# shuoshuof/Humanoid-Real-Time-Retarget

Measured on AMD Instinct MI355X. Metric: retargeted frames/sec + max joint-angle err vs ref, Hu humanoid @1/2/4/8 GPU, higher is better.
Workload: dtype f32; 1 GPU; VtrdynFullBodyPosRetargeter batched solve, Hu v5 target (BASELINE config 3); global_batch=262144, parallelism=dp1, input_layout=soa, input_ring_sets=3, precise_gripper=True, launch=K plain launches, step i on stream i % 2

## Files before the change

humanoid-real-time-retarget_amd/csrc/rtg_knobs.h:

```cpp
#pragma once

#ifndef RTG_SIDES_TILES
#define RTG_SIDES_TILES 2
#endif
#ifndef RTG_SIDES_EARLY_WORDS
#define RTG_SIDES_EARLY_WORDS 1
#endif
#ifndef RTG_AOS_PRELOAD_TIPS
#define RTG_AOS_PRELOAD_TIPS 1
#endif
#ifndef RTG_SIDES_SOA_WAVES
#define RTG_SIDES_SOA_WAVES 5
#endif
#ifndef RTG_SIDES_UNIFORM_WAVE
#define RTG_SIDES_UNIFORM_WAVE 3
#endif
#ifndef RTG_QUAD8_MAX_B
#define RTG_QUAD8_MAX_B 2048
#endif
#ifndef RTG_QUAD_MAX_B
#define RTG_QUAD_MAX_B 4096
#endif
#ifndef RTG_LATENCY_MAX_B
#define RTG_LATENCY_MAX_B 49152
#endif
#ifndef RTG_EXP_HOT_INPUTS
#define RTG_EXP_HOT_INPUTS 0
#endif
#ifndef RTG_EXP_TIMESTAMPS
#define RTG_EXP_TIMESTAMPS 0
#endif
#ifndef RTG_EXP_SKIP_SIGNAL
#define RTG_EXP_SKIP_SIGNAL 0
#endif
#ifndef RTG_VEL_SEG
#define RTG_VEL_SEG 10
#endif
#ifndef RTG_VEL_LDS_MIN
#define RTG_VEL_LDS_MIN 0
#endif
#ifndef RTG_FK_NT_OUT
#define RTG_FK_NT_OUT 1
#endif
#ifndef RTG_FK_F16_MAXJ
#define RTG_FK_F16_MAXJ 36
#endif
#ifndef RTG_EXP_MULR_NOBRANCH
#define RTG_EXP_MULR_NOBRANCH 0
#endif
#ifndef RTG_EXP_NO_TABLE
#define RTG_EXP_NO_TABLE 0
#endif
#ifndef RTG_TORSO_X0
#define RTG_TORSO_X0 1
#endif
#ifndef RTG_FIT_FAST_DIV
#define RTG_FIT_FAST_DIV 1
#endif
#ifndef RTG_FIT_FAST_DIV_TU
#define RTG_FIT_FAST_DIV_TU RTG_FIT_FAST_DIV
#endif
#ifndef RTG_FDIV_CORRECTIONS
#define RTG_FDIV_CORRECTIONS 1
#endif
#if RTG_FDIV_CORRECTIONS != 1 && RTG_FDIV_CORRECTIONS != 2
#error "RTG_FDIV_CORRECTIONS: 1 or 2 (fewer gives wrong quotients)"
#endif
#ifndef RTG_DOF_NT_STORE
#define RTG_DOF_NT_STORE 1
#endif
#ifndef RTG_VEL_W
#define RTG_VEL_W 8
#endif
#ifndef RTG_DOF_NWAY
#define RTG_DOF_NWAY 4
#endif
#ifndef RTG_UNIT_TAB_K
#define RTG_UNIT_TAB_K 16
#endif
#ifndef RTG_SIDES_SHARED_FIT
#define RTG_SIDES_SHARED_FIT 1
#endif
#ifndef RTG_EULER_LIBM
#define RTG_EULER_LIBM 1
#endif
#ifndef RTG_UPPER_UNIT_TAB
#define RTG_UPPER_UNIT_TAB 1
#endif
#ifndef RTG_ROT_UNIT_TAB
#define RTG_ROT_UNIT_TAB 1
#endif
#ifndef RTG_SIDES_UNIT_TAB
#define RTG_SIDES_UNIT_TAB 7
#endif
#ifndef RTG_SIDES_UNIT_TAB_AOS
#define RTG_SIDES_UNIT_TAB_AOS 1
#endif
#ifndef RTG_FRAME1_UNIT_TAB
#define RTG_FRAME1_UNIT_TAB 6
#endif
#ifndef RTG_FK_UNIT_TAB
#define RTG_FK_UNIT_TAB 1
#endif
#ifndef RTG_DOF_UNIT_TAB
#define RTG_DOF_UNIT_TAB 1
#endif
#ifndef RTG_VEL_UNIT_TAB
#define RTG_VEL_UNIT_TAB 1
#endif
#ifndef RTG_VEL_ANG_NB
#define RTG_VEL_ANG_NB 2
#endif
#ifndef RTG_ROT_INGEST_TILE_AOS
#define RTG_ROT_INGEST_TILE_AOS 16
#endif
#ifndef RTG_ROT_INGEST_TILE_SOA
#define RTG_ROT_INGEST_TILE_SOA 16
#endif
#ifndef RTG_EXP_NO_RARE
#define RTG_EXP_NO_RARE 0
#endif
#ifndef RTG_EXP_STUB_SVD
#define RTG_EXP_STUB_SVD 0
#endif
```

humanoid-real-time-retarget_amd/csrc/rtg_ops.hip:

```cpp
#include "rtg_device.cuh"

namespace rtg {

struct Dir3 {
    float x, y, z;
    int32_t on;
};

__global__ __launch_bounds__(256) void k_rescale_motion(TopoView T, const float *__restrict__ motion, int64_t B,
                                                        Dir3 dir, float *__restrict__ out)
{
    const int64_t f = (int64_t)blockIdx.x * blockDim.x + threadIdx.x;
    if (f >= B) return;
    const int J = T.J;
    const float *m = motion + f * J * 3;
    float *o = out + f * J * 3;
    auto mp = [&](int j) {
        const V v = ld3(m + 3 * j);
        return dir.on ? V{v.x * dir.x, v.y * dir.y, v.z * dir.z} : v;
    };
    for (int j = 0; j < J; ++j) {
        const int p = ld_const(T.parents + j);
        const V mj = mp(j);
        if (p < 0) {
// ... 760 lines not shown
    for (int i = 0; i < 20; ++i) {
#pragma unroll
        for (int c = 0; c < 3; ++c) {
            lh[lay_idx(soa, f, i, c, 20, 3, B)] = jit(14 + i, c);
            rh[lay_idx(soa, f, i, c, 20, 3, B)] = jit(39 + i, c);
        }
    }
}

hipError_t launch_rescale_motion(const TopoView &T, const float *motion, int64_t B, const float *dir, float *out,
                                 hipStream_t s)
{
    const Dir3 d = dir ? Dir3{dir[0], dir[1], dir[2], 1} : Dir3{1.0f, 1.0f, 1.0f, 0};
    hipLaunchKernelGGL(k_rescale_motion, dim3(grid_for(B, 256)), dim3(256), 0, s, T, motion, B, d, out);
    return hipGetLastError();
}

hipError_t launch_quat_between(const float *v1, const float *v2, int64_t n, float *out, float *ws, hipStream_t s)
{
    hipError_t e = hipMemsetAsync(ws, 0, 2 * sizeof(float), s);
    if (e != hipSuccess) return e;
    hipLaunchKernelGGL(k_qbtv_norm_max, dim3(grid_for(n, 256)), dim3(256), 0, s, v1, v2, n, ws);
    hipLaunchKernelGGL(k_quat_between, dim3(grid_for(n, 256)), dim3(256), 0, s, v1, v2, n, ws, out);
    return hipGetLastError();
}

hipError_t launch_rebuild_vtrdyn(const TopoView &T, const float *motion, int64_t B, float *g_rot, float *root_t,
                                 float *ws, hipStream_t s)
{
    hipError_t e = hipMemsetAsync(ws, 0, T.J * sizeof(float), s);
    if (e != hipSuccess) return e;
    hipLaunchKernelGGL(k_rebuild_norm_max, dim3(grid_for(B, 256)), dim3(256), 0, s, T, motion, B, ws);
    hipLaunchKernelGGL(k_rebuild_vtrdyn, dim3(grid_for(B, 256)), dim3(256), 0, s, T, motion, B, ws, g_rot, root_t);
    return hipGetLastError();
}

hipError_t launch_ingest_vtrdyn(const float *bp, const float *lhp, const float *rhp, int64_t B, int layout,
                                float *body, float *lh, float *rh, uint8_t *valid, hipStream_t s)
{
    if (layout == RTG_LAYOUT_SOA)
        hipLaunchKernelGGL(k_ingest_vtrdyn<kIngSoaTile>, dim3(grid_for(B, kIngSoaTile)), dim3(256), 0, s, bp,
                           lhp, rhp, B, body, lh, rh, valid, true);
    else
        hipLaunchKernelGGL(k_ingest_vtrdyn<kIngAosTile>, dim3(grid_for(B, kIngAosTile)), dim3(256), 0, s, bp,
                           lhp, rhp, B, body, lh, rh, valid, false);
    return hipGetLastError();
}

hipError_t launch_quat_op(int op, const float *a, const float *b, const float *c, int64_t n, float *out,
                          hipStream_t s)
{
    hipLaunchKernelGGL(k_quat_op, dim3(grid_for(n, 256)), dim3(256), 0, s, op, a, b, c, n, out);
    return hipGetLastError();
}

hipError_t launch_cal_joint_quat(const float *Z, const float *M, int npts, int64_t n, float *out, hipStream_t s)
{
    const dim3 g(grid_for(n, 256)), b(256);
    switch (npts) {
    case 1: hipLaunchKernelGGL(k_cal_joint_quat<1>, g, b, 0, s, Z, M, n, out); break;
    case 2: hipLaunchKernelGGL(k_cal_joint_quat<2>, g, b, 0, s, Z, M, n, out); break;
    case 3: hipLaunchKernelGGL(k_cal_joint_quat<3>, g, b, 0, s, Z, M, n, out); break;
    case 4: hipLaunchKernelGGL(k_cal_joint_quat<4>, g, b, 0, s, Z, M, n, out); break;
    case 5: hipLaunchKernelGGL(k_cal_joint_quat<5>, g, b, 0, s, Z, M, n, out); break;
    case 6: hipLaunchKernelGGL(k_cal_joint_quat<6>, g, b, 0, s, Z, M, n, out); break;
    case 7: hipLaunchKernelGGL(k_cal_joint_quat<7>, g, b, 0, s, Z, M, n, out); break;
    default: hipLaunchKernelGGL(k_cal_joint_quat<8>, g, b, 0, s, Z, M, n, out); break;
    }
    return hipGetLastError();
}

hipError_t launch_quat_as_euler(const float *q, int s0, int s1, int s2, int extrinsic, int degrees, int64_t n,
                               double *out, hipStream_t s)
{
    hipLaunchKernelGGL(k_quat_as_euler, dim3(grid_for(n, 256)), dim3(256), 0, s, q, s0, s1, s2, extrinsic, degrees, n,
                       out);
    return hipGetLastError();
}
hipError_t launch_quat_in_xyz_axis(const float *q, int s0, int s1, int s2, int extrinsic, int64_t n, float *out,
                                   hipStream_t s)
{
    hipLaunchKernelGGL(k_quat_in_xyz_axis, dim3(grid_for(n, 256)), dim3(256), 0, s, q, s0, s1, s2, extrinsic, n, out);
    return hipGetLastError();
}

hipError_t launch_synth_full_body(const TopoView &T, uint64_t seed, int64_t off, int64_t B, float *body, float *lh,
                                  float *rh, float *body_rot, int layout, hipStream_t s)
{
    hipLaunchKernelGGL(k_synth_full_body, dim3(grid_for(B, 64)), dim3(64), 0, s, T, seed, off, B, body, lh, rh,
                       body_rot,
                       layout == RTG_LAYOUT_SOA);
    return hipGetLastError();
}

constexpr int kProbeIters = 4096;
__global__ __launch_bounds__(256) void k_probe_valu(float seed, float *__restrict__ sink, uint64_t *__restrict__ clk)
{
    float a[8];
#pragma unroll
    for (int k = 0; k < 8; ++k) a[k] = seed + (float)(threadIdx.x + k);
    const bool rec = (blockIdx.x & 63) == 0 && threadIdx.x == 0;
    uint64_t c0 = 0, w0 = 0;
    if (rec) {
        c0 = clock64();
        w0 = wall_clock64();
    }
    for (int i = 0; i < kProbeIters; ++i) {
#pragma unroll
        for (int k = 0; k < 8; ++k) a[k] = __builtin_fmaf(a[k], 0.999999f, 1e-7f);
    }
    if (rec) {
        const uint64_t c1 = clock64(), w1 = wall_clock64();
        clk[2 * (blockIdx.x >> 6)] = c1 - c0;
        clk[2 * (blockIdx.x >> 6) + 1] = w1 - w0;
    }
    float s = 0.0f;
#pragma unroll
    for (int k = 0; k < 8; ++k) s += a[k];
    if (s == 12345.678f) sink[threadIdx.x] = s;
}
__global__ __launch_bounds__(256) void k_probe_copy(const float4 *__restrict__ src, float4 *__restrict__ dst,
                                                    int64_t n)
{
    for (int64_t i = (int64_t)blockIdx.x * 256 + threadIdx.x; i < n; i += (int64_t)gridDim.x * 256) dst[i] = src[i];
}

hipError_t launch_probe_valu(int nblocks, float *sink, uint64_t *clk, hipStream_t s)
{
    hipLaunchKernelGGL(k_probe_valu, dim3(nblocks), dim3(256), 0, s, 1.0f, sink, clk);
    return hipGetLastError();
}
hipError_t launch_probe_copy(const float *src, float *dst, int64_t nfloat4, hipStream_t s)
{
    hipLaunchKernelGGL(k_probe_copy, dim3(256 * 32), dim3(256), 0, s, reinterpret_cast<const float4 *>(src),
                       reinterpret_cast<float4 *>(dst), nfloat4);
    return hipGetLastError();
}
int probe_valu_iters() { return kProbeIters; }

}

#if RTG_EXP_STUB_SVD + RTG_EXP_NO_TABLE + RTG_EXP_HOT_INPUTS + RTG_EXP_MULR_NOBRANCH + RTG_EXP_NO_RARE + \
    RTG_EXP_TIMESTAMPS + RTG_EXP_SKIP_SIGNAL == 0
#define RTG_WRONG_ANSWER_KNOBS 0
#else
#define RTG_WRONG_ANSWER_KNOBS 1
#endif
#define RTG_STR2(x) #x
#define RTG_STR(x) RTG_STR2(x)
#define RTG_KNOB(k) "\"" #k "\":\"" RTG_STR(k) "\","
extern "C" const char *rtg_build_info(void)
{
    return "{\"abi\":" RTG_STR(RTG_ABI_VERSION) ",\"arch\":\"gfx950\",\"knobs\":{"
        RTG_KNOB(RTG_DOF_NWAY) RTG_KNOB(RTG_DOF_UNIT_TAB) RTG_KNOB(RTG_FK_UNIT_TAB) RTG_KNOB(RTG_UNIT_TAB_K) RTG_KNOB(RTG_SIDES_SHARED_FIT) RTG_KNOB(RTG_UPPER_UNIT_TAB) RTG_KNOB(RTG_ROT_UNIT_TAB) RTG_KNOB(RTG_EULER_LIBM) RTG_KNOB(RTG_SIDES_UNIT_TAB) RTG_KNOB(RTG_SIDES_UNIT_TAB_AOS) RTG_KNOB(RTG_FRAME1_UNIT_TAB) RTG_KNOB(RTG_VEL_UNIT_TAB) RTG_KNOB(RTG_SIDES_SOA_WAVES) RTG_KNOB(RTG_SIDES_UNIFORM_WAVE) RTG_KNOB(RTG_SIDES_TILES) RTG_KNOB(RTG_SIDES_EARLY_WORDS) RTG_KNOB(RTG_AOS_PRELOAD_TIPS) RTG_KNOB(RTG_QUAD8_MAX_B) RTG_KNOB(RTG_QUAD_MAX_B) RTG_KNOB(RTG_LATENCY_MAX_B)
        RTG_KNOB(RTG_EXP_TIMESTAMPS) RTG_KNOB(RTG_EXP_SKIP_SIGNAL) RTG_KNOB(RTG_EXP_STUB_SVD) RTG_KNOB(RTG_EXP_NO_TABLE) RTG_KNOB(RTG_EXP_MULR_NOBRANCH) RTG_KNOB(RTG_FK_F16_MAXJ) RTG_KNOB(RTG_FK_NT_OUT) RTG_KNOB(RTG_TORSO_X0) RTG_KNOB(RTG_VEL_SEG) RTG_KNOB(RTG_VEL_LDS_MIN) RTG_KNOB(RTG_DOF_NT_STORE) RTG_KNOB(RTG_VEL_W) RTG_KNOB(RTG_VEL_ANG_NB) RTG_KNOB(RTG_EXP_NO_RARE)
        RTG_KNOB(RTG_ROT_INGEST_TILE_AOS) RTG_KNOB(RTG_ROT_INGEST_TILE_SOA) RTG_KNOB(RTG_FIT_FAST_DIV) RTG_KNOB(RTG_FIT_FAST_DIV_TU) RTG_KNOB(RTG_FDIV_CORRECTIONS)
        "\"RTG_EXP_HOT_INPUTS\":\"" RTG_STR(RTG_EXP_HOT_INPUTS) "\"},\"wrong_answer_knobs\":"
        RTG_STR(RTG_WRONG_ANSWER_KNOBS) "}";
}
```

humanoid-real-time-retarget_amd/csrc/rtg_solver.cuh:

```cuda
#pragma once
#include "rtg_device.cuh"

namespace rtg {

struct Emit {
    float *row;
    float *__restrict__ lr;
    const uint32_t *__restrict__ ang;
    float2 *st;
    int sst;
    uint32_t *wd = nullptr;
    template <int LINK>
    static constexpr int slot() { return LINK <= 18 ? LINK - 12 : LINK - 14; }
    RTG_DEV void load_word(int s, float w) const
    {
#if !RTG_EXP_NO_TABLE
        __builtin_amdgcn_global_load_lds((const __attribute__((address_space(1))) void *)(ang + ang_tab_word_of(w)),
                                         (__attribute__((address_space(3))) void *)(wd + s * 64), 4, 0, 0);
#endif
    }
    template <int LINK>
    RTG_DEV void link(Q q) const
    {
        constexpr int k = hu_dof_axis(LINK - 1);
        st[slot<LINK>() * sst] = make_float2(q.w, k == 0 ? q.x : (k == 1 ? q.y : q.z));
        if (wd) load_word(slot<LINK>(), q.w);
        if (lr) st4(lr + 4 * LINK, q);
    }
    template <int LINK>
    RTG_DEV void identity() const
    {
        st[slot<LINK>() * sst] = make_float2(1.0f, 0.0f);
        if (lr) st4(lr + 4 * LINK, qident());
    }
    RTG_DEV void finalize(int s0, int n) const
    {
        uint32_t exact = 0;
        if (wd) wait_words();
#pragma unroll
        for (int j = 0; j < 14; ++j)
            if (j >= s0 && j < s0 + n) {
                const float2 v = st[j * sst];
                const ExpDof e = wd ? exp_dof_word_part(v.x, wd[j * 64 + (threadIdx.x & 63)]) : exp_dof_table_part(v.x, ang);
                exact |= (uint32_t)e.exact << j;
                row[j < 7 ? 11 + j : 13 + j] = exp_dof_finish(e, v.y);
            }
        if (__builtin_expect(exact != 0u, 0)) {
#pragma unroll 1
            for (int j = s0; j < s0 + n; ++j)
                if ((exact >> j) & 1u) {
                    const float2 v = st[j * sst];
                    row[j < 7 ? 11 + j : 13 + j] = exp_dof_exact(v.x, v.y);
                }
        }
    }
    static RTG_DEV void wait_words() { __builtin_amdgcn_s_waitcnt(0x0F70); }
};

RTG_DEV void emit_fixed_links(const Emit &E, bool write_lr = true, int k0 = 0)
{
#pragma unroll
    for (int k = 0; k < 11; ++k)
        if (k >= k0) E.row[k] = 0.0f;
    E.row[29] = 0.0f;
    if (E.lr && write_lr) {
#pragma unroll
        for (int j = 0; j < 12; ++j) st4(E.lr + 4 * j, qident());
        st4(E.lr + 4 * 19, qident());
        st4(E.lr + 4 * 20, qident());
        st4(E.lr + 4 * 28, qident());
        st4(E.lr + 4 * 29, qident());
        st4(E.lr + 4 * 30, qident());
    }
}

enum : uint32_t {
    kStTorsoSvd = 1,
    kStLeftSvd = 2,
    kStLeftEuler = 4,
    kStRightSvd = 8,
    kStRightEuler = 16,
};
RTG_DEV uint32_t frame_error_code(uint32_t bits)
{
    const uint32_t first = bits & (0u - bits);
    return (first & (kStTorsoSvd | kStLeftSvd | kStRightSvd)) ? RTG_FRAME_SVD_NONFINITE : RTG_FRAME_ZERO_NORM_QUAT;
}
RTG_DEV void poison_frame(float *drow, float *__restrict__ lr, float *__restrict__ br, uint32_t bits)
{
    const float qn = __builtin_bit_cast(float, RTG_FRAME_NAN);
    drow[0] = __builtin_bit_cast(float, RTG_FRAME_NAN | frame_error_code(bits));
#pragma unroll
    for (int k = 1; k < 30; ++k) drow[k] = qn;
    const Q qq{qn, qn, qn, qn};
    if (lr)
        for (int j = 0; j < 31; ++j) st4(lr + 4 * j, qq);
    if (br)
        for (int j = 0; j < 59; ++j) st4(br + 4 * j, qq);
}

RTG_DEV void report_device_error(uint32_t *err, uint32_t code)
{
    if (err) __hip_atomic_fetch_or(err, code, __ATOMIC_RELAXED, __HIP_MEMORY_SCOPE_SYSTEM);
}

template <int L0, typename Tab = NoTab>
RTG_DEV Q solve_arm(const Emit &E, V upper, V fore, ArmZero zs, ArmZero ze, Q parent, Tab tab = Tab{})
{
    Q p, r, y, e;
    shoulder_pr(upper, zs, parent, p, r, tab);
    E.link<L0>(p);
    E.link<L0 + 1>(r);
    elbow_py(fore, ze, qmul(qmul(parent, p), r), y, e, tab);
    E.link<L0 + 2>(y);
    E.link<L0 + 3>(e);
    return qmul(qmul(qmul(p, r), y), e);
}

RTG_DEV void link_rt(const Emit &E, int link, Q q)
{
    const int k = kHuDofAxis[link - 1];
    E.st[(link <= 18 ? link - 12 : link - 14) * E.sst] = make_float2(q.w, k == 0 ? q.x : (k == 1 ? q.y : q.z));
    if (E.lr) st4(E.lr + 4 * link, q);
}
template <int L0>
RTG_DEV bool emit_euler_xyz(const Emit &E, Q local)
{
    Q eul[3];
    const bool refused = quat_in_xyz_intrinsic(local, eul);
    E.link<L0>(eul[0]);
    E.link<L0 + 1>(eul[1]);
    E.link<L0 + 2>(eul[2]);
    return refused;
}

RTG_DEV float hand_x_mean(Q rot, V h0, const V (&tip)[5])
{
    const float x0 = qrotate(rot, h0).x;
    return mean5(qrotate(rot, tip[0]).x - x0, qrotate(rot, tip[1]).x - x0, qrotate(rot, tip[2]).x - x0,
                 qrotate(rot, tip[3]).x - x0, qrotate(rot, tip[4]).x - x0);
}
template <bool SOA>
struct FV;
template <>
struct FV<false> {
    const float *__restrict__ p;
    RTG_DEV V p3(int j) const { return ld3(p + 3 * j); }
    RTG_DEV Q q4(int j) const { return ld4(p + 4 * j); }
};
template <>
struct FV<true> {
    const float *__restrict__ p;
    int64_t s;
    RTG_DEV float e(int64_t i) const { return p[i]; }
    RTG_DEV V p3(int j) const { return V{e((3 * j) * s), e((3 * j + 1) * s), e((3 * j + 2) * s)}; }
    RTG_DEV Q q4(int j) const { return Q{e((4 * j) * s), e((4 * j + 1) * s), e((4 * j + 2) * s), e((4 * j + 3) * s)}; }
};
template <bool SOA>
RTG_DEV FV<SOA> frame_view(const float *__restrict__ base, int64_t f, int row_floats, int64_t B);
template <>
RTG_DEV FV<false> frame_view<false>(const float *__restrict__ base, int64_t f, int row_floats, int64_t)
{
    return FV<false>{base + f * row_floats};
}
template <>
RTG_DEV FV<true> frame_view<true>(const float *__restrict__ base, int64_t f, int, int64_t B)
{
    return FV<true>{base + f, B};
}

template <typename View>
RTG_DEV float hand_x_mean(Q rot, const View &H, const int (&idx)[5])
{
    const V tip[5] = {H.p3(idx[0]), H.p3(idx[1]), H.p3(idx[2]), H.p3(idx[3]), H.p3(idx[4])};
    return hand_x_mean(rot, H.p3(0), tip);
}

constexpr int kDofStride = 31;

RTG_DEV void store_dof_rows(float *__restrict__ dst, const float *src, int64_t nrows, int t, int nthr)
{
    const int nvals = (int)nrows * 30;
    auto at = [&](int i) {
        const int rr = i / 30;
        return src[rr * kDofStride + (i - rr * 30)];
    };
    const int nvec = nvals >> 2;
    typedef float f4v __attribute__((ext_vector_type(4)));
    const int dr = (4 * nthr) / 30, dc = (4 * nthr) - dr * 30;
    int rr = (4 * t) / 30, c = 4 * t - rr * 30;
    for (int v = t; v < nvec; v += nthr) {
        const int i = v << 2;
        const float *p = src + rr * kDofStride + c;
        const int wrap = c == 28 ? 1 : 0;
        const f4v q = {p[0], p[1], p[2 + wrap], p[3 + wrap]};
        if (RTG_DOF_NT_STORE) __builtin_nontemporal_store(q, reinterpret_cast<f4v *>(dst + i));
        else *reinterpret_cast<f4v *>(dst + i) = q;
        c += dc;
        rr += dr;
        if (c >= 30) { c -= 30; ++rr; }
    }
    for (int i = (nvec << 2) + t; i < nvals; i += nthr) dst[i] = at(i);
}

constexpr int kSideTiles = RTG_SIDES_TILES;
constexpr int kSideThreads = 128 * kSideTiles;
constexpr int kSideFrames = 64 * kSideTiles;

template <typename View, typename Hook = NoHook, typename Tab = NoTab>
RTG_DEV Q fbp_torso(const SolverConsts &C, const View &b, bool &svd_nan, const Hook &hook = Hook{}, Tab tab = Tab{})
{
    const V b10 = b.p3(10);
    const V Mt[3] = {vsub(b.p3(17), b10), vsub(b.p3(13), b10), vsub(b.p3(11), b10)};
    return cal_joint_quat<3>(C.Zt, Mt, svd_nan, hook, tab);
}
RTG_DEV Q upper_pt_sign(V v) { return Q{v.x * -1.0f, v.y * -1.0f, v.z * 1.0f, 0.0f}; }
template <typename View>
RTG_DEV Q upper_torso(const SolverConsts &C, const View &x, bool &svd_nan)
{
    auto pt = [&](int j) {
        const Q q = upper_pt_sign(x.p3(j));
        return V{q.x, q.y, q.z};
    };
    const V s10 = pt(10);
    const V Mt[3] = {vsub(pt(17), s10), vsub(pt(13), s10), vsub(pt(11), s10)};
    return cal_joint_quat<3>(C.Zt, Mt, svd_nan);
}
template <int SIDE, typename View, typename Hook = NoHook, typename Tab = NoTab>
RTG_DEV Q fbp_wrist_fit(const SolverConsts &C, const View &H, bool &svd_nan, const Hook &hook = Hook{}, Tab tab = Tab{})
{
    const V h0 = H.p3(0);
    const V M[5] = {vsub(H.p3(2), h0), vsub(H.p3(6), h0), vsub(H.p3(10), h0), vsub(H.p3(14), h0), vsub(H.p3(17), h0)};
    return cal_joint_quat<5>(SIDE ? C.Zr : C.Zl, M, svd_nan, hook, tab);
}
struct ArmPts { V sh, el, wr; };
struct TipPts { V h0, t[5]; };
template <int SIDE, typename View>
RTG_DEV ArmPts load_arm(const View &b)
{
    return ArmPts{b.p3(SIDE ? 14 : 18), b.p3(SIDE ? 15 : 19), b.p3(SIDE ? 16 : 20)};
}
template <typename View>
RTG_DEV TipPts load_tips(const View &H)
{
    return TipPts{H.p3(0), {H.p3(4), H.p3(8), H.p3(12), H.p3(16), H.p3(19)}};
}

template <typename Tab = NoTab>
RTG_DEV void fbp_arms2(const SolverConsts &C, const ArmPts &apL, const ArmPts &apR, Q R10, const Emit &E, Q &chL,
                       Q &chR, Tab tab = Tab{})
{
    const V up[2] = {vsub(apL.el, apL.sh), vsub(apR.el, apR.sh)};
    const V fo[2] = {vsub(apL.wr, apL.el), vsub(apR.wr, apR.el)};
    const ArmZero zs[2] = {C.lsh, C.rsh}, ze[2] = {C.lel, C.rel};
    const Q par[2] = {R10, R10};
    Q p[2], r[2], y[2], e[2];
    arm_pair_n<true, 2>(up, zs, par, p, r, tab);
    E.link<12>(p[0]);
    E.link<13>(r[0]);
    E.link<21>(p[1]);
    E.link<22>(r[1]);
    const Q par2[2] = {qmul(qmul(R10, p[0]), r[0]), qmul(qmul(R10, p[1]), r[1])};
    arm_pair_n<false, 2>(fo, ze, par2, y, e, tab);
    E.link<14>(y[0]);
    E.link<15>(e[0]);
    E.link<23>(y[1]);
    E.link<24>(e[1]);
    chL = qmul(qmul(qmul(p[0], r[0]), y[0]), e[0]);
    chR = qmul(qmul(qmul(p[1], r[1]), y[1]), e[1]);
}
template <bool PRECISE>
RTG_DEV void fbp_gripper(const SolverConsts &C, float a, float *row_d0)
{
    if (PRECISE) {
        const float sc = clamp_lohi(a / C.orig - 0.5f, 0.0f, 0.5f) / 0.5f;
        row_d0[0] = sc * 0.044f;
        row_d0[1] = sc * -0.044f;
    } else {
        const bool closed = a / C.orig < 0.7f;
        row_d0[0] = closed ? 0.0f : 0.044f;
        row_d0[1] = closed ? 0.0f : -0.044f;
    }
}
template <int SIDE>
RTG_DEV void fbp_body_rows(float *__restrict__ brow, Q R10, Q W, bool const_rows = true)
{
    st4(brow + 4 * (SIDE ? 39 : 14), W);
    if (!SIDE) {
        if (const_rows) {
            for (int j = 0; j < 59; ++j)
                if (j != 14 && j != 39) st4(brow + 4 * j, j == 10 ? R10 : qident());
        } else {
            st4(brow + 4 * 10, R10);
        }
    }
}
template <bool PRECISE, int SIDE, typename Tab = NoTab>
RTG_DEV bool fbp_side_after_arm(const SolverConsts &C, const TipPts &tp, Q R10, Q chain, Q W, const Emit &E,
                                float *__restrict__ brow, Tab tab = Tab{})
{
    constexpr int E0 = SIDE ? 25 : 16, D0 = SIDE ? 27 : 18;
    const bool refused = emit_euler_xyz<E0>(E, qmul_norm(qconj(qmul_norm(R10, chain, tab)), W, tab));
    fbp_gripper<PRECISE>(C, hand_x_mean(qconj(W), tp.h0, tp.t), E.row + D0);
    if (brow) fbp_body_rows<SIDE>(brow, R10, W);
    return refused;
}

template <int SIDE, typename View, typename Tab = NoTab>
RTG_DEV void solve_upper_side(const SolverConsts &C, const View &x, Q R10, const Emit &E, Tab tab = Tab{})
{
    auto pt = [&](int j) {
        const Q q = upper_pt_sign(x.p3(j));
        return V{q.x, q.y, q.z};
    };
    constexpr int L0 = SIDE ? 21 : 12, E0 = SIDE ? 25 : 16, D0 = SIDE ? 27 : 18;
    constexpr int SH = SIDE ? 14 : 18, EL = SIDE ? 15 : 19, WR = SIDE ? 16 : 20;
    const V sel = pt(EL);
    solve_arm<L0>(E, vsub(sel, pt(SH)), vsub(pt(WR), sel), SIDE ? C.rsh : C.lsh, SIDE ? C.rel : C.lel, R10, tab);
    E.identity<E0>(); E.identity<E0 + 1>(); E.identity<E0 + 2>();
    E.row[D0] = 0.0f; E.row[D0 + 1] = 0.0f;
}

template <int SIDE, typename View, typename Tab = NoTab>
RTG_DEV bool solve_full_body_rot_side(const SolverConsts &C, const View &q, const View &b, const View &H,
                                      const Emit &E, Tab tab = Tab{})
{
    constexpr int L0 = SIDE ? 21 : 12, E0 = SIDE ? 25 : 16, D0 = SIDE ? 27 : 18;
    constexpr int SH = SIDE ? 14 : 18, EL = SIDE ? 15 : 19, WR = SIDE ? 16 : 20, PAR = SIDE ? 13 : 17;
    const Q par = q.q4(PAR);
    const V bel = b.p3(EL);
    const Q chain = solve_arm<L0>(E, vsub(bel, b.p3(SH)), vsub(b.p3(WR), bel), SIDE ? C.rsh : C.lsh,
                                  SIDE ? C.rel : C.lel, par, tab);
    const Q w = q.q4(WR);
    const bool refused = emit_euler_xyz<E0>(E, qmul_norm(qconj(qmul_norm(par, chain, tab)), w, tab));
    constexpr int tips[5] = {3, 7, 11, 15, 19};
    const bool closed = hand_x_mean(w, H, tips) / C.orig < 0.7f;
    E.row[D0] = closed ? 0.0f : 0.044f;
    E.row[D0 + 1] = closed ? 0.0f : -0.044f;
    return refused;
}

template <int SIDE, typename View, typename Tab = NoTab>
RTG_DEV bool solve_body_rot_side(const SolverConsts &C, const View &g, const Emit &E, Tab tab = Tab{})
{
    auto local = [&](int j, int p) { return qmul_norm(qconj(g.q4(p)), g.q4(j), tab); };
    constexpr int SH = SIDE ? 14 : 18, EL = SIDE ? 15 : 19, D0 = SIDE ? 27 : 18;
    Q s3[3], e3[3];
    bool refused = quat_in_xyz_axis(local(SH, C.par[SIDE ? 1 : 0]), 1, 0, 2, false, s3);
    refused |= quat_in_xyz_axis(local(EL, C.par[SIDE ? 3 : 2]), 2, 1, 0, false, e3);
    if (SIDE) {
        E.link<21>(s3[0]); E.link<22>(s3[1]); E.link<23>(qmul_norm(e3[0], s3[2], tab));
        E.link<24>(e3[1]); E.link<25>(e3[2]);
        E.identity<26>(); E.identity<27>();
    } else {
        E.link<12>(s3[0]); E.link<13>(s3[1]); E.link<14>(qmul_norm(e3[0], s3[2], tab));
        E.link<15>(e3[1]); E.link<16>(e3[2]);
        E.identity<17>(); E.identity<18>();
    }
    E.row[D0] = 0.0f; E.row[D0 + 1] = 0.0f;
    return refused;
}

RTG_DEV void lds_signal(int *flag)
{
    __builtin_amdgcn_fence(__ATOMIC_RELEASE, "workgroup");
    const uint64_t joined = __builtin_amdgcn_ballot_w64(true);
    if (joined != 0 && (threadIdx.x & 63) == (unsigned)__builtin_ctzll(joined))
        __hip_atomic_store(flag, 1, __ATOMIC_RELEASE, __HIP_MEMORY_SCOPE_WORKGROUP);
}
RTG_DEV void lds_wait(int *flag, uint32_t *err)
{
    for (int it = 0; it < (1 << 22); ++it) {
        if (__hip_atomic_load(flag, __ATOMIC_ACQUIRE, __HIP_MEMORY_SCOPE_WORKGROUP)) return;
        __builtin_amdgcn_s_sleep(1);
    }
    if ((threadIdx.x & 63) == 0) report_device_error(err, RTG_DEVERR_HANDOVER_TIMEOUT);
}

constexpr int kSlotDwords = 4;
RTG_DEV void slot_put(float *row, Q q) { row[0] = q.x; row[1] = q.y; row[2] = q.z; row[3] = q.w; }
RTG_DEV Q slot_get(const float *row) { return Q{row[0], row[1], row[2], row[3]}; }
RTG_DEV void slot_clear(float *row) { row[0] = 0.0f; row[1] = 0.0f; row[2] = 0.0f; row[3] = 0.0f; }

template <int KIND, bool SOA>
constexpr int side_min_waves() { return KIND == RTG_SOLVER_FULL_BODY_POS && SOA ? RTG_SIDES_SOA_WAVES : 1; }
constexpr int kSideLdsBudgetSoa = 32000 * kSideTiles / 2;

template <int KIND, bool PRECISE, bool SOA>
__global__ __launch_bounds__(kSideThreads, (side_min_waves<KIND, SOA>())) void k_solve_sides(
                                                     SolverConsts C, const float *__restrict__ in0,
                                                     const float *__restrict__ in1, const float *__restrict__ in2,
                                                     const float *__restrict__ in3, int64_t B,
                                                     float *__restrict__ dof, float *__restrict__ local_rot,
                                                     float *__restrict__ body_rot)
{
    __shared__ float sdof[kSideFrames * kDofStride];
    __shared__ float2 sst[kSideTiles * 14 * 64];
    __shared__ uint8_t sstat[2][kSideFrames];
    constexpr bool kUniformWave = (RTG_SIDES_UNIFORM_WAVE & (KIND != RTG_SOLVER_FULL_BODY_POS ? 4 : (SOA ? 1 : 2))) != 0;
    const int w = kUniformWave ? __builtin_amdgcn_readfirstlane(threadIdx.x >> 6) : (int)(threadIdx.x >> 6);
    const int side = w & 1, lane = threadIdx.x & 63;
    const int r = (w >> 1) * 64 + lane;
    const int64_t f0 = (int64_t)blockIdx.x * kSideFrames, f = f0 + r;
    const bool live = f < B;
    float *const lrow = live && local_rot ? local_rot + f * 124 : nullptr;
#if RTG_SIDES_EARLY_WORDS
    __shared__ uint32_t swd[kSideTiles * 14 * 64];
    uint32_t *const wds = KIND == RTG_SOLVER_FULL_BODY_POS && !SOA ? swd + (w >> 1) * 14 * 64 : nullptr;
#else
    uint32_t *const wds = nullptr;
#endif
    const Emit E{sdof + r * kDofStride, lrow, C.ang_tab, sst + (w >> 1) * 14 * 64 + lane, 64, wds};
#if RTG_EXP_HOT_INPUTS
    const int64_t fi = f & (kSideFrames - 1);
#else
    const int64_t fi = f;
#endif
    auto view = [&](const float *base, int row_floats) { return frame_view<SOA>(base, fi, row_floats, B); };
#if RTG_EXP_TIMESTAMPS
    float *const tsb = body_rot;
    body_rot = nullptr;
    auto TS = [&](int k) {
        if (tsb && (blockIdx.x & 7) == 0 && lane == 0) {
            const uint64_t t = wall_clock64();
            uint32_t *o = reinterpret_cast<uint32_t *>(tsb) + 2 * (((blockIdx.x >> 3) * (2 * kSideTiles) + w) * 16 + k);
            o[0] = (uint32_t)t;
            o[1] = (uint32_t)(t >> 32);
        }
    };
#else
    auto TS = [](int) {};
#endif
    uint32_t st = 0;
    bool fit1_nan = false, fit2_nan = false, euler_refused = false;
    if constexpr (KIND == RTG_SOLVER_FULL_BODY_POS) {
        __shared__ int sflag[kSideTiles][4];
        if (threadIdx.x < 4 * kSideTiles) (&sflag[0][0])[threadIdx.x] = 0;
        constexpr int kTab = SOA ? RTG_SIDES_UNIT_TAB : RTG_SIDES_UNIT_TAB_AOS;
        __shared__ UnitEnt sut[2 * kUnitTabK + 1];
        if constexpr (kTab != 0) unit_tab_fill(sut, (int)threadIdx.x);
        static_assert(!SOA || sizeof(sdof) + sizeof(sst) + sizeof(sstat) + sizeof(sflag) + sizeof(sut) <= kSideLdsBudgetSoa,
                      "the SoA FULL_BODY_POS side kernel's LDS no longer lets five blocks share a CU");
        const auto tabF = TabSel<(kTab & 1) != 0>::get(sut);
        const auto tabA = TabSel<(kTab & 2) != 0>::get(sut);
        const auto tabE = TabSel<(kTab & 4) != 0>::get(sut);
        __syncthreads();
        int *const fl = sflag[w >> 1];
        auto hook1 = [&](int k) { if (k < 2) TS(1 + k); };
        auto hook2 = [&](int k) { if (k < 2) TS(10 + k); };
        TS(0);
        const auto b = view(in0, 63);
        Q R10 = qident(), W = qident();
        ArmPts apL{}, apR{};
        constexpr bool kPreTips = RTG_AOS_PRELOAD_TIPS && !SOA;
        TipPts tpre{};
        constexpr bool kSharedFit = RTG_SIDES_SHARED_FIT >= (SOA ? 1 : 2);
        constexpr bool kTorsoX0 = RTG_TORSO_X0 && !RTG_EXP_STUB_SVD;
        if (live) {
            if constexpr (kSharedFit) {
                float A[9];
                Q q = qident();
                bool general = true;
                if (!side) {
                    const V b10 = b.p3(10);
                    const V Mt[3] = {vsub(b.p3(17), b10), vsub(b.p3(13), b10), vsub(b.p3(11), b10)};
                    if constexpr (kTorsoX0) {
                        if (C.torso_x0) general = !torso_quat_x0(C.Zt, Mt, q, hook1, tabF);
                    }
                    if (general) fit1_nan = form_joint_A<3>(C.Zt, Mt, A);
                } else {
                    apL = load_arm<0>(b);
                    apR = load_arm<1>(b);
                    const auto H = view(in2, 60);
                    if (kPreTips) tpre = load_tips(H);
                    const V h0 = H.p3(0);
                    const V M[5] = {vsub(H.p3(2), h0), vsub(H.p3(6), h0), vsub(H.p3(10), h0), vsub(H.p3(14), h0),
                                    vsub(H.p3(17), h0)};
                    fit1_nan = form_joint_A<5>(C.Zr, M, A);
                }
                if (general) q = joint_quat_of_A(A, hook1, tabF);
                if (!side) {
                    R10 = q;
                    slot_put(E.row, R10);
                } else {
                    W = q;
                }
            } else {
                bool nan = false;
                if (!side) {
                    bool general = true;
                    if constexpr (kTorsoX0) {
                        if (C.torso_x0) {
                            const V b10 = b.p3(10);
                            const V Mt[3] = {vsub(b.p3(17), b10), vsub(b.p3(13), b10), vsub(b.p3(11), b10)};
                            general = !torso_quat_x0(C.Zt, Mt, R10, hook1, tabF);
                        }
                    }
                    if (general) R10 = fbp_torso(C, b, nan, hook1, tabF);
                    slot_put(E.row, R10);
                    fit1_nan = nan;
                } else {
                    apL = load_arm<0>(b);
                    apR = load_arm<1>(b);
                    if (kPreTips) tpre = load_tips(view(in2, 60));
                    W = fbp_wrist_fit<1>(C, view(in2, 60), nan, hook1, tabF);
                    fit1_nan = nan;
                }
            }
        }
        TS(3);
        if (!side) {
            if (!(RTG_EXP_SKIP_SIGNAL && blockIdx.x == 0 && w == 0)) lds_signal(&fl[0]);
        } else {
            lds_wait(&fl[0], C.err);
        }
        TS(4);
        Q chain = qident();
        if (side) {
            if (live) {
                R10 = slot_get(E.row);
                Q cl;
                fbp_arms2(C, apL, apR, R10, E, cl, chain, tabA);
                slot_put(E.row, cl);
            }
            if (wds) Emit::wait_words();
            lds_signal(&fl[1]);
        } else if (live) {
            emit_fixed_links(E, true, kSlotDwords);
            bool nan = false;
            if (kPreTips) tpre = load_tips(view(in1, 60));
            W = fbp_wrist_fit<0>(C, view(in1, 60), nan, hook2, tabF);
            fit2_nan = nan;
        }
        TS(5);
        if (!side) lds_wait(&fl[1], C.err);
        TS(6);
        if (live) {
            float *brow = body_rot ? body_rot + f * 236 : nullptr;
            const TipPts tp = kPreTips ? tpre : load_tips(view(side ? in2 : in1, 60));
            if (side) {
                euler_refused = fbp_side_after_arm<PRECISE, 1>(C, tp, R10, chain, W, E, brow, tabE);
            } else {
                const Q c = slot_get(E.row);
                slot_clear(E.row);
                euler_refused = fbp_side_after_arm<PRECISE, 0>(C, tp, R10, c, W, E, brow, tabE);
            }
        }
        TS(7);
        if (live) E.finalize(side ? 7 : 0, 7);
        st = side ? ((fit1_nan ? kStRightSvd : 0u) | (euler_refused ? kStRightEuler : 0u))
                  : ((fit1_nan ? kStTorsoSvd : 0u) | (fit2_nan ? kStLeftSvd : 0u) | (euler_refused ? kStLeftEuler : 0u));
        sstat[side][r] = (uint8_t)st;
        TS(8);
        __builtin_amdgcn_fence(__ATOMIC_RELEASE, "workgroup");
        const uint64_t joined = __builtin_amdgcn_ballot_w64(true);
        const int first = __builtin_ctzll(joined);
        int prev = 0;
        if (lane == first) prev = __hip_atomic_fetch_add(&fl[2], 1, __ATOMIC_RELAXED, __HIP_MEMORY_SCOPE_WORKGROUP);
        if (__builtin_amdgcn_readlane(prev, first) == 0) {
            TS(9);
            TS(12);
            return;
        }
        __builtin_amdgcn_fence(__ATOMIC_ACQUIRE, "workgroup");
        TS(9);
        const int64_t t0 = f0 + (w >> 1) * 64;
        const int64_t nrows = (B - t0) < 64 ? (B - t0) : 64;
        if (nrows <= 0) return;
        float *const tile = sdof + (w >> 1) * 64 * kDofStride;
        const uint32_t bits = live ? (uint32_t)(sstat[0][r] | sstat[1][r]) : 0u;
        if (__builtin_amdgcn_ballot_w64(bits != 0u)) {
            if (bits) {
                const int64_t fr = t0 + lane;
                poison_frame(tile + lane * kDofStride, local_rot ? local_rot + fr * 124 : nullptr,
                             body_rot ? body_rot + fr * 236 : nullptr, bits);
            }
            __builtin_amdgcn_fence(__ATOMIC_SEQ_CST, "workgroup");
        }
        store_dof_rows(dof + t0 * 30, tile, nrows, lane, 64);
        TS(12);
        return;
    } else {
        TS(0);
        if constexpr (KIND == RTG_SOLVER_UPPER_BODY) {
            const auto b = view(in0, 63);
            Q R10 = qident();
            __shared__ UnitEnt sut[2 * kUnitTabK + 1];
            if (RTG_UPPER_UNIT_TAB && side) unit_tab_fill(sut, lane);
            const auto tab = TabSel<RTG_UPPER_UNIT_TAB != 0>::get(sut);
            if (live && !side) {
                bool nan = false;
                R10 = upper_torso(C, b, nan);
                slot_put(E.row, R10);
                st |= nan ? kStTorsoSvd : 0u;
            }
            __syncthreads();
            if (live) {
                if (side) {
                    R10 = slot_get(E.row);
                    slot_clear(E.row);
                    solve_upper_side<1>(C, b, R10, E, tab);
                } else {
                    emit_fixed_links(E, true, kSlotDwords);
                    solve_upper_side<0>(C, b, R10, E, tab);
                }
            }
        } else {
            constexpr bool kRotTab = RTG_ROT_UNIT_TAB && KIND == RTG_SOLVER_FULL_BODY_ROT;
            __shared__ UnitEnt sutw[2 * kSideTiles][2 * kUnitTabK + 1];
            if (kRotTab) {
                unit_tab_fill(sutw[w], lane);
                __builtin_amdgcn_fence(__ATOMIC_RELEASE, "wavefront");
                __builtin_amdgcn_wave_barrier();
                __builtin_amdgcn_fence(__ATOMIC_ACQUIRE, "wavefront");
            }
            const auto tab = TabSel<kRotTab>::get(sutw[w]);
            if (live) {
                if (!side) emit_fixed_links(E);
                bool refused;
                if constexpr (KIND == RTG_SOLVER_FULL_BODY_ROT) {
                    refused = side ? solve_full_body_rot_side<1>(C, view(in0, 84), view(in1, 63), view(in3, 60), E, tab)
                                   : solve_full_body_rot_side<0>(C, view(in0, 84), view(in1, 63), view(in2, 60), E, tab);
                } else {
                    refused = side ? solve_body_rot_side<1>(C, view(in0, 84), E, tab)
                                   : solve_body_rot_side<0>(C, view(in0, 84), E, tab);
                }
                st |= refused ? (side ? kStRightEuler : kStLeftEuler) : 0u;
            }
        }
        if (live) E.finalize(side ? 7 : 0, 7);
        sstat[side][r] = (uint8_t)st;
        TS(8);
        __syncthreads();
        TS(9);
        const uint32_t bits = (live && !side) ? (uint32_t)(sstat[0][r] | sstat[1][r]) : 0u;
        if (__syncthreads_or(bits != 0u)) {
            if (bits) poison_frame(E.row, lrow, nullptr, bits);
            __syncthreads();
        }
        const int64_t nrows = (B - f0) < kSideFrames ? (B - f0) : kSideFrames;
        store_dof_rows(dof + f0 * 30, sdof, nrows, threadIdx.x, kSideThreads);
        TS(12);
    }
}

constexpr int kLatFrames = 64;

template <bool PRECISE, bool SOA>
RTG_DEV void fbp_latency5_tile(const SolverConsts &C, const float *__restrict__ in0, const float *__restrict__ in1,
                               const float *__restrict__ in2, int64_t B, int64_t f0, float *__restrict__ dof,
                               float *__restrict__ local_rot, float *__restrict__ body_rot)
{
    __shared__ float sdof[kLatFrames * kDofStride];
    __shared__ float4 sfit[kLatFrames];
    __shared__ float4 schain[2][kLatFrames];
    __shared__ float2 sst[14 * kLatFrames];
    __shared__ int sflag[3];
    __shared__ uint8_t sstat[3][kLatFrames];
    const int w = threadIdx.x >> 6, lane = threadIdx.x & 63;
    const int64_t f = f0 + lane;
    const bool live = f < B;
    if (threadIdx.x < 3) sflag[threadIdx.x] = 0;
    __syncthreads();
#if RTG_EXP_TIMESTAMPS
    float *const tsb = body_rot;
    body_rot = nullptr;
    auto TS = [&](int k) {
        if (tsb && blockIdx.x == 0 && lane == 0) {
            const uint64_t t = wall_clock64();
            reinterpret_cast<uint32_t *>(tsb)[2 * (16 * w + k)] = (uint32_t)t;
            reinterpret_cast<uint32_t *>(tsb)[2 * (16 * w + k) + 1] = (uint32_t)(t >> 32);
        }
    };
#else
    auto TS = [](int) {};
#endif
    auto hook = [&](int k) { if (k < 2) TS(8 + k); };
    TS(0);
    float *const lrow = live && local_rot ? local_rot + f * 124 : nullptr;
    const Emit E{sdof + lane * kDofStride, lrow, C.ang_tab, sst + lane, kLatFrames};
    auto view = [&](const float *base, int row_floats) { return frame_view<SOA>(base, f, row_floats, B); };
    const auto b = view(in0, 63);
    bool fit_nan = false, euler_refused = false;
    if (w == 0) {
        if (live) {
            bool nan = false;
            const Q q = fbp_torso(C, b, nan, hook);
            sfit[lane] = make_float4(q.x, q.y, q.z, q.w);
            fit_nan = nan;
        }
        lds_signal(&sflag[0]);
        TS(1);
        if (live) emit_fixed_links(E);
        TS(2);
    } else if (w >= 3) {
        const int side = w - 3;
        ArmPts ap{};
        if (live) ap = side ? load_arm<1>(b) : load_arm<0>(b);
        TS(1);
        lds_wait(&sflag[0], C.err);
        TS(2);
        if (live) {
            const float4 t = sfit[lane];
            const Q R10{t.x, t.y, t.z, t.w};
// ... 549 lines not shown
```

Before: 4.586 billion frames/s.

## Rebalance sides kernel so each wave solves its own arm and wrist

```diff
diff --git a/humanoid-real-time-retarget_amd/csrc/rtg_knobs.h b/humanoid-real-time-retarget_amd/csrc/rtg_knobs.h
--- a/humanoid-real-time-retarget_amd/csrc/rtg_knobs.h
+++ b/humanoid-real-time-retarget_amd/csrc/rtg_knobs.h
@@ -78,9 +78,6 @@
 #ifndef RTG_UNIT_TAB_K
 #define RTG_UNIT_TAB_K 16
 #endif
-#ifndef RTG_SIDES_SHARED_FIT
-#define RTG_SIDES_SHARED_FIT 1
-#endif
 #ifndef RTG_EULER_LIBM
 #define RTG_EULER_LIBM 1
 #endif
diff --git a/humanoid-real-time-retarget_amd/csrc/rtg_ops.hip b/humanoid-real-time-retarget_amd/csrc/rtg_ops.hip
--- a/humanoid-real-time-retarget_amd/csrc/rtg_ops.hip
+++ b/humanoid-real-time-retarget_amd/csrc/rtg_ops.hip
@@ -936,7 +936,7 @@
 extern "C" const char *rtg_build_info(void)
 {
     return "{\"abi\":" RTG_STR(RTG_ABI_VERSION) ",\"arch\":\"gfx950\",\"knobs\":{"
-        RTG_KNOB(RTG_DOF_NWAY) RTG_KNOB(RTG_DOF_UNIT_TAB) RTG_KNOB(RTG_FK_UNIT_TAB) RTG_KNOB(RTG_UNIT_TAB_K) RTG_KNOB(RTG_SIDES_SHARED_FIT) RTG_KNOB(RTG_UPPER_UNIT_TAB) RTG_KNOB(RTG_ROT_UNIT_TAB) RTG_KNOB(RTG_EULER_LIBM) RTG_KNOB(RTG_SIDES_UNIT_TAB) RTG_KNOB(RTG_SIDES_UNIT_TAB_AOS) RTG_KNOB(RTG_FRAME1_UNIT_TAB) RTG_KNOB(RTG_VEL_UNIT_TAB) RTG_KNOB(RTG_SIDES_SOA_WAVES) RTG_KNOB(RTG_SIDES_UNIFORM_WAVE) RTG_KNOB(RTG_SIDES_TILES) RTG_KNOB(RTG_SIDES_EARLY_WORDS) RTG_KNOB(RTG_AOS_PRELOAD_TIPS) RTG_KNOB(RTG_QUAD8_MAX_B) RTG_KNOB(RTG_QUAD_MAX_B) RTG_KNOB(RTG_LATENCY_MAX_B)
+        RTG_KNOB(RTG_DOF_NWAY) RTG_KNOB(RTG_DOF_UNIT_TAB) RTG_KNOB(RTG_FK_UNIT_TAB) RTG_KNOB(RTG_UNIT_TAB_K) RTG_KNOB(RTG_UPPER_UNIT_TAB) RTG_KNOB(RTG_ROT_UNIT_TAB) RTG_KNOB(RTG_EULER_LIBM) RTG_KNOB(RTG_SIDES_UNIT_TAB) RTG_KNOB(RTG_SIDES_UNIT_TAB_AOS) RTG_KNOB(RTG_FRAME1_UNIT_TAB) RTG_KNOB(RTG_VEL_UNIT_TAB) RTG_KNOB(RTG_SIDES_SOA_WAVES) RTG_KNOB(RTG_SIDES_UNIFORM_WAVE) RTG_KNOB(RTG_SIDES_TILES) RTG_KNOB(RTG_SIDES_EARLY_WORDS) RTG_KNOB(RTG_AOS_PRELOAD_TIPS) RTG_KNOB(RTG_QUAD8_MAX_B) RTG_KNOB(RTG_QUAD_MAX_B) RTG_KNOB(RTG_LATENCY_MAX_B)
         RTG_KNOB(RTG_EXP_TIMESTAMPS) RTG_KNOB(RTG_EXP_SKIP_SIGNAL) RTG_KNOB(RTG_EXP_STUB_SVD) RTG_KNOB(RTG_EXP_NO_TABLE) RTG_KNOB(RTG_EXP_MULR_NOBRANCH) RTG_KNOB(RTG_FK_F16_MAXJ) RTG_KNOB(RTG_FK_NT_OUT) RTG_KNOB(RTG_TORSO_X0) RTG_KNOB(RTG_VEL_SEG) RTG_KNOB(RTG_VEL_LDS_MIN) RTG_KNOB(RTG_DOF_NT_STORE) RTG_KNOB(RTG_VEL_W) RTG_KNOB(RTG_VEL_ANG_NB) RTG_KNOB(RTG_EXP_NO_RARE)
         RTG_KNOB(RTG_ROT_INGEST_TILE_AOS) RTG_KNOB(RTG_ROT_INGEST_TILE_SOA) RTG_KNOB(RTG_FIT_FAST_DIV) RTG_KNOB(RTG_FIT_FAST_DIV_TU) RTG_KNOB(RTG_FDIV_CORRECTIONS)
         "\"RTG_EXP_HOT_INPUTS\":\"" RTG_STR(RTG_EXP_HOT_INPUTS) "\"},\"wrong_answer_knobs\":"
diff --git a/humanoid-real-time-retarget_amd/csrc/rtg_solver.cuh b/humanoid-real-time-retarget_amd/csrc/rtg_solver.cuh
--- a/humanoid-real-time-retarget_amd/csrc/rtg_solver.cuh
+++ b/humanoid-real-time-retarget_amd/csrc/rtg_solver.cuh
@@ -55,7 +55,17 @@
         }
     }
     static RTG_DEV void wait_words() { __builtin_amdgcn_s_waitcnt(0x0F70); }
+    RTG_DEV Emit shifted(int dl, int ds) const
+    {
+        return Emit{row + dl, lr ? lr + 4 * dl : nullptr, ang, st + ds * sst, sst, wd ? wd + ds * 64 : nullptr};
+    }
 };
+constexpr bool side_links_alike(int a, int b, int n)
+{
+    for (int j = 0; j < n; ++j)
+        if (hu_dof_axis(a + j - 1) != hu_dof_axis(b + j - 1)) return false;
+    return true;
+}
 
 RTG_DEV void emit_fixed_links(const Emit &E, bool write_lr = true, int k0 = 0)
 {
@@ -246,29 +256,6 @@
     return TipPts{H.p3(0), {H.p3(4), H.p3(8), H.p3(12), H.p3(16), H.p3(19)}};
 }
 
-template <typename Tab = NoTab>
-RTG_DEV void fbp_arms2(const SolverConsts &C, const ArmPts &apL, const ArmPts &apR, Q R10, const Emit &E, Q &chL,
-                       Q &chR, Tab tab = Tab{})
-{
-    const V up[2] = {vsub(apL.el, apL.sh), vsub(apR.el, apR.sh)};
-    const V fo[2] = {vsub(apL.wr, apL.el), vsub(apR.wr, apR.el)};
-    const ArmZero zs[2] = {C.lsh, C.rsh}, ze[2] = {C.lel, C.rel};
-    const Q par[2] = {R10, R10};
-    Q p[2], r[2], y[2], e[2];
-    arm_pair_n<true, 2>(up, zs, par, p, r, tab);
-    E.link<12>(p[0]);
-    E.link<13>(r[0]);
-    E.link<21>(p[1]);
-    E.link<22>(r[1]);
-    const Q par2[2] = {qmul(qmul(R10, p[0]), r[0]), qmul(qmul(R10, p[1]), r[1])};
-    arm_pair_n<false, 2>(fo, ze, par2, y, e, tab);
-    E.link<14>(y[0]);
-    E.link<15>(e[0]);
-    E.link<23>(y[1]);
-    E.link<24>(e[1]);
-    chL = qmul(qmul(qmul(p[0], r[0]), y[0]), e[0]);
-    chR = qmul(qmul(qmul(p[1], r[1]), y[1]), e[1]);
-}
 template <bool PRECISE>
 RTG_DEV void fbp_gripper(const SolverConsts &C, float a, float *row_d0)
 {
@@ -294,16 +281,6 @@
             st4(brow + 4 * 10, R10);
         }
     }
-}
-template <bool PRECISE, int SIDE, typename Tab = NoTab>
-RTG_DEV bool fbp_side_after_arm(const SolverConsts &C, const TipPts &tp, Q R10, Q chain, Q W, const Emit &E,
-                                float *__restrict__ brow, Tab tab = Tab{})
-{
-    constexpr int E0 = SIDE ? 25 : 16, D0 = SIDE ? 27 : 18;
-    const bool refused = emit_euler_xyz<E0>(E, qmul_norm(qconj(qmul_norm(R10, chain, tab)), W, tab));
-    fbp_gripper<PRECISE>(C, hand_x_mean(qconj(W), tp.h0, tp.t), E.row + D0);
-    if (brow) fbp_body_rows<SIDE>(brow, R10, W);
-    return refused;
 }
 
 template <int SIDE, typename View, typename Tab = NoTab>
@@ -432,7 +409,7 @@
     auto TS = [](int) {};
 #endif
     uint32_t st = 0;
-    bool fit1_nan = false, fit2_nan = false, euler_refused = false;
+    bool torso_nan = false, wrist_nan = false, euler_refused = false;
     if constexpr (KIND == RTG_SOLVER_FULL_BODY_POS) {
         __shared__ int sflag[kSideTiles][4];
         if (threadIdx.x < 4 * kSideTiles) (&sflag[0][0])[threadIdx.x] = 0;
@@ -446,110 +423,72 @@
         const auto tabE = TabSel<(kTab & 4) != 0>::get(sut);
         __syncthreads();
         int *const fl = sflag[w >> 1];
-        auto hook1 = [&](int k) { if (k < 2) TS(1 + k); };
-        auto hook2 = [&](int k) { if (k < 2) TS(10 + k); };
+        auto hookT = [&](int k) { if (k < 2) TS(1 + k); };
+        auto hookW = [&](int k) { if (k < 2) TS((side ? 1 : 10) + k); };
         TS(0);
         const auto b = view(in0, 63);
+        static_assert(Emit::slot<21>() - Emit::slot<12>() == 7 && side_links_alike(12, 21, 7), "the sides' links differ");
+        const Emit ES = E.shifted(side ? 9 : 0, side ? 7 : 0);
+        V Z[5];
+#pragma unroll
+        for (int t = 0; t < 5; ++t) Z[t] = side ? C.Zr[t] : C.Zl[t];
+        const ArmZero zsh = side ? C.rsh : C.lsh, zel = side ? C.rel : C.lel;
+        const auto H = view(side ? in2 : in1, 60);
+        const int jsh = side ? 14 : 18;
         Q R10 = qident(), W = qident();
-        ArmPts apL{}, apR{};
         constexpr bool kPreTips = RTG_AOS_PRELOAD_TIPS && !SOA;
         TipPts tpre{};
-        constexpr bool kSharedFit = RTG_SIDES_SHARED_FIT >= (SOA ? 1 : 2);
         constexpr bool kTorsoX0 = RTG_TORSO_X0 && !RTG_EXP_STUB_SVD;
+        ArmPts ap{};
+        if (live) ap = ArmPts{b.p3(jsh), b.p3(jsh + 1), b.p3(jsh + 2)};
+        if (!side) {
+            if (live) {
+                const V b10 = b.p3(10);
+                const V Mt[3] = {vsub(b.p3(17), b10), vsub(b.p3(13), b10), vsub(b.p3(11), b10)};
+                bool general = true;
+                if constexpr (kTorsoX0) {
+                    if (C.torso_x0) general = !torso_quat_x0(C.Zt, Mt, R10, hookT, tabF);
+                }
+                if (general) R10 = cal_joint_quat<3>(C.Zt, Mt, torso_nan, hookT, tabF);
+                slot_put(E.row, R10);
+            }
+            TS(3);
+            if (!(RTG_EXP_SKIP_SIGNAL && blockIdx.x == 0 && w == 0)) lds_signal(&fl[0]);
+            TS(4);
+            if (live) emit_fixed_links(E, true, kSlotDwords);
+        }
         if (live) {
-            if constexpr (kSharedFit) {
-                float A[9];
-                Q q = qident();
-                bool general = true;
-                if (!side) {
-                    const V b10 = b.p3(10);
-                    const V Mt[3] = {vsub(b.p3(17), b10), vsub(b.p3(13), b10), vsub(b.p3(11), b10)};
-                    if constexpr (kTorsoX0) {
-                        if (C.torso_x0) general = !torso_quat_x0(C.Zt, Mt, q, hook1, tabF);
-                    }
-                    if (general) fit1_nan = form_joint_A<3>(C.Zt, Mt, A);
-                } else {
-                    apL = load_arm<0>(b);
-                    apR = load_arm<1>(b);
-                    const auto H = view(in2, 60);
-                    if (kPreTips) tpre = load_tips(H);
-                    const V h0 = H.p3(0);
-                    const V M[5] = {vsub(H.p3(2), h0), vsub(H.p3(6), h0), vsub(H.p3(10), h0), vsub(H.p3(14), h0),
-                                    vsub(H.p3(17), h0)};
-                    fit1_nan = form_joint_A<5>(C.Zr, M, A);
-                }
-                if (general) q = joint_quat_of_A(A, hook1, tabF);
-                if (!side) {
-                    R10 = q;
-                    slot_put(E.row, R10);
-                } else {
-                    W = q;
-                }
-            } else {
-                bool nan = false;
-                if (!side) {
-                    bool general = true;
-                    if constexpr (kTorsoX0) {
-                        if (C.torso_x0) {
-                            const V b10 = b.p3(10);
-                            const V Mt[3] = {vsub(b.p3(17), b10), vsub(b.p3(13), b10), vsub(b.p3(11), b10)};
-                            general = !torso_quat_x0(C.Zt, Mt, R10, hook1, tabF);
-                        }
-                    }
-                    if (general) R10 = fbp_torso(C, b, nan, hook1, tabF);
-                    slot_put(E.row, R10);
-                    fit1_nan = nan;
-                } else {
-                    apL = load_arm<0>(b);
-                    apR = load_arm<1>(b);
-                    if (kPreTips) tpre = load_tips(view(in2, 60));
-                    W = fbp_wrist_fit<1>(C, view(in2, 60), nan, hook1, tabF);
-                    fit1_nan = nan;
-                }
-            }
-        }
-        TS(3);
-        if (!side) {
-            if (!(RTG_EXP_SKIP_SIGNAL && blockIdx.x == 0 && w == 0)) lds_signal(&fl[0]);
-        } else {
+            if (kPreTips) tpre = load_tips(H);
+            const V h0 = H.p3(0);
+            const V M[5] = {vsub(H.p3(2), h0), vsub(H.p3(6), h0), vsub(H.p3(10), h0), vsub(H.p3(14), h0), vsub(H.p3(17), h0)};
+            W = cal_joint_quat<5>(Z, M, wrist_nan, hookW, tabF);
+        }
+        if (side) {
+            TS(3);
             lds_wait(&fl[0], C.err);
-        }
-        TS(4);
-        Q chain = qident();
-        if (side) {
+            TS(4);
             if (live) {
                 R10 = slot_get(E.row);
-                Q cl;
-                fbp_arms2(C, apL, apR, R10, E, cl, chain, tabA);
-                slot_put(E.row, cl);
-            }
-            if (wds) Emit::wait_words();
-            lds_signal(&fl[1]);
-        } else if (live) {
-            emit_fixed_links(E, true, kSlotDwords);
-            bool nan = false;
-            if (kPreTips) tpre = load_tips(view(in1, 60));
-            W = fbp_wrist_fit<0>(C, view(in1, 60), nan, hook2, tabF);
-            fit2_nan = nan;
-        }
-        TS(5);
-        if (!side) lds_wait(&fl[1], C.err);
-        TS(6);
+                slot_clear(E.row);
+            }
+        }
         if (live) {
-            float *brow = body_rot ? body_rot + f * 236 : nullptr;
-            const TipPts tp = kPreTips ? tpre : load_tips(view(side ? in2 : in1, 60));
-            if (side) {
-                euler_refused = fbp_side_after_arm<PRECISE, 1>(C, tp, R10, chain, W, E, brow, tabE);
-            } else {
-                const Q c = slot_get(E.row);
-                slot_clear(E.row);
-                euler_refused = fbp_side_after_arm<PRECISE, 0>(C, tp, R10, c, W, E, brow, tabE);
+            const Q chain = solve_arm<12>(ES, vsub(ap.el, ap.sh), vsub(ap.wr, ap.el), zsh, zel, R10, tabA);
+            TS(5);
+            TS(6);
+            const TipPts tp = kPreTips ? tpre : load_tips(H);
+            euler_refused = emit_euler_xyz<16>(ES, qmul_norm(qconj(qmul_norm(R10, chain, tabE)), W, tabE));
+            fbp_gripper<PRECISE>(C, hand_x_mean(qconj(W), tp.h0, tp.t), ES.row + 18);
+            if (body_rot) {
+                float *brow = body_rot + f * 236;
+                if (side) fbp_body_rows<1>(brow, R10, W);
+                else fbp_body_rows<0>(brow, R10, W);
             }
         }
         TS(7);
-        if (live) E.finalize(side ? 7 : 0, 7);
-        st = side ? ((fit1_nan ? kStRightSvd : 0u) | (euler_refused ? kStRightEuler : 0u))
-                  : ((fit1_nan ? kStTorsoSvd : 0u) | (fit2_nan ? kStLeftSvd : 0u) | (euler_refused ? kStLeftEuler : 0u));
+        if (live) ES.finalize(0, 7);
+        st = side ? ((wrist_nan ? kStRightSvd : 0u) | (euler_refused ? kStRightEuler : 0u))
+                  : ((torso_nan ? kStTorsoSvd : 0u) | (wrist_nan ? kStLeftSvd : 0u) | (euler_refused ? kStLeftEuler : 0u));
         sstat[side][r] = (uint8_t)st;
         TS(8);
         __builtin_amdgcn_fence(__ATOMIC_RELEASE, "workgroup");
```

Result: faster. 4.714 billion frames/s (median of 6 runs) (+2.8%).
